# colinvaz/nmf-toolbox

Measured on AMD Instinct MI355X. Metric: NMF multiplicative-update iterations/s, higher is better.
Workload: dtype f32; 1 GPU; nmf.m kl MU, V=16384x65536 K=256 fp32, V column-sharded over 1 GPU(s); m=16384, n=65536, K=256, T=1, divergence=kl

## Files before the change

### nmf_toolbox_amd/build.py

```python
from __future__ import annotations

import os
import subprocess
import sys
from concurrent.futures import ThreadPoolExecutor

HERE = os.path.dirname(os.path.abspath(__file__))
CSRC = os.path.join(HERE, "csrc")
INC = os.path.join(os.path.dirname(HERE), "include")
OUT = os.path.join(HERE, "libnmfx.so")
SOURCES = ["fused_cnmf_a.hip", "fused_cnmf_b.hip", "fused_cnmf_c.hip", "fused_cnmf_e.hip", "fused_cnmf_d.hip", "fused_cnmf_g.hip", "fused_cnmf_f.hip", "gemm_pipe_edge.hip", "gemm_pipe.hip", "gemm.hip", "fused_k224_256.hip", "fused_rag_k224_256.hip", "fused_k128_192.hip", "fused_rag_k128_192.hip", "fused_k32_96.hip", "fused_rag_k32_96.hip", "fused.hip", "aux.hip", "projfunc.hip", "small_mm.hip", "gemm64.hip", "engine.hip", "host_io.hip", "blocking.hip", "sc.hip", "sc64.hip", "multi_sc.hip", "rccl_backend.hip", "cmfwisa.hip", "seminmf.hip"]
ARCH = "gfx950"


def _torch_lib_dir():
    try:
        import importlib.util
        spec = importlib.util.find_spec("torch")
        if spec and spec.origin:
            d = os.path.join(os.path.dirname(spec.origin), "lib")
            if os.path.exists(os.path.join(d, "libamdhip64.so")):
                return d
    except Exception:
        pass
    return None


def _deps(src, incdirs, seen=None):
    import re
    seen = set() if seen is None else seen
    if src in seen or not os.path.exists(src):
        return seen
    seen.add(src)
    with open(src) as f:
        for name in re.findall(r'^\s*#\s*include\s*"([^"]+)"', f.read(), re.M):
            for d in [os.path.dirname(src)] + incdirs:
                cand = os.path.join(d, name)
                if os.path.exists(cand):
                    _deps(cand, incdirs, seen)
                    break
    return seen


def _newer(src_list, target):
    if not os.path.exists(target):
        return True
    t = os.path.getmtime(target)
    return any(os.path.getmtime(s) > t for s in src_list)


VARIANTS = {
    "r5": ["-DNMFX_KL_MODE=0", "-DNMFX_G2_VEC=0", "-DNMFX_G1_ASM=0"],
    "kl1": ["-DNMFX_KL_MODE=1", "-DNMFX_G2_VEC=0", "-DNMFX_G1_ASM=0"],
    "kl2": ["-DNMFX_KL_MODE=2", "-DNMFX_G2_VEC=0", "-DNMFX_G1_ASM=0"],
    "kl2g2": ["-DNMFX_KL_MODE=2", "-DNMFX_G2_VEC=1", "-DNMFX_G1_ASM=0"],
}


def build(force: bool = False, verbose: bool = False, sanitize: bool = False, variant: str = "") -> str:
    srcs = [os.path.join(CSRC, s) for s in SOURCES if os.path.exists(os.path.join(CSRC, s))]
    objdir = os.path.join(CSRC, "_obj_asan" if sanitize else ("_obj_" + variant if variant else "_obj"))
    out = os.path.join(HERE, "libnmfx_asan.so") if sanitize else (os.path.join(HERE, "libnmfx_%s.so" % variant) if variant else OUT)
    vdefs = VARIANTS[variant] if variant else []
    san = ["-fsanitize=address,undefined", "-fno-sanitize=function", "-fno-gpu-sanitize", "-fno-sanitize-recover=undefined", "-Xarch_host", "-g", "-Xarch_host", "-fno-omit-frame-pointer"] if sanitize else []
    os.makedirs(objdir, exist_ok=True)
    hipcc = os.environ.get("HIPCC", "/opt/rocm/bin/hipcc")

    def compile_one(src):
        obj = os.path.join(objdir, os.path.basename(src) + ".o")
        if force or _newer(sorted(_deps(src, [CSRC, INC])) + [os.path.abspath(__file__)], obj):
            cmd = [hipcc, f"--offload-arch={ARCH}", "-O3", "-std=c++17", "-fPIC", "-Wall", "-Werror=uninitialized", "-Wno-pass-failed"] + san + vdefs + [
                   "-I", INC, "-I", CSRC, "-c", src, "-o", obj]
            if os.path.basename(src).startswith("fused_"):
                cmd[3:3] = ["-mllvm", "-pragma-unroll-threshold=1000000"]
            if verbose:
                print(" ".join(cmd), flush=True)
            subprocess.check_call(cmd)
        return obj

    with ThreadPoolExecutor(max_workers=min(len(srcs), 8)) as ex:
        objs = list(ex.map(compile_one, srcs))
    if force or _newer(objs, out):
        tl = _torch_lib_dir()
        libdirs = ([tl] if tl else []) + ["/opt/rocm/lib"]
        if sanitize:
            cmd = ["/opt/rocm/lib/llvm/bin/clang++", "-shared", "-fsanitize=address,undefined", "-fno-sanitize=function", "-o", out] + objs
        else:
            cmd = ["g++", "-shared", "-o", out] + objs
# ... 34 lines not shown
```

### nmf_toolbox_amd/csrc/fused_kernel.h

```cpp
#pragma once
#include "nmfx_internal.h"

namespace nmfx {

typedef float f32x16 __attribute__((ext_vector_type(16)));
typedef float f32x2 __attribute__((ext_vector_type(2)));

typedef int i32x4 __attribute__((ext_vector_type(4)));

constexpr int FT_ROWS = 128;
constexpr int FT_C = 64;

__device__ __forceinline__ f32x2 pk_mul_t(f32x2 a, f32x2 b) { f32x2 d; asm("s_nop 0\n\tv_pk_mul_f32 %0, %1, %2" : "=v"(d) : "v"(a), "v"(b)); return d; }
__device__ __forceinline__ f32x2 pk_fma_t(f32x2 a, f32x2 b, f32x2 c) { f32x2 d; asm("s_nop 0\n\tv_pk_fma_f32 %0, %1, %2, %3" : "=v"(d) : "v"(a), "v"(b), "v"(c)); return d; }
__device__ __forceinline__ f32x2 pk_fnma(f32x2 a, f32x2 b, f32x2 c) { f32x2 d; asm("v_pk_fma_f32 %0, %1, %2, %3 neg_lo:[1,0,0] neg_hi:[1,0,0]" : "=v"(d) : "v"(a), "v"(b), "v"(c)); return d; }
__device__ __forceinline__ f32x2 pk_add(f32x2 a, f32x2 b) { f32x2 d; asm("v_pk_add_f32 %0, %1, %2" : "=v"(d) : "v"(a), "v"(b)); return d; }

__device__ __forceinline__ void mfma_settle_full(f32x16 &t) { asm volatile("s_nop 15\n\ts_nop 3" : "+v"(t)); }
__device__ __forceinline__ constexpr int rowmap(int reg, int h) { return (reg & 3) + 8 * (reg >> 2) + 4 * h; }
__device__ __forceinline__ i32x4 make_srd(const void *base, unsigned bytes) {
    const unsigned long long b = (unsigned long long)base;
    i32x4 s;
    s.x = (int)(unsigned)b;
    s.y = (int)((b >> 32) & 0xffffu);
    s.z = (int)bytes;
    s.w = 0x00020000;
    return s;
}

template <int K, bool D_RC, int FUNC, bool DO_G2, int EPI, bool RAG = false, int TT = 1>
__global__ __launch_bounds__(256, ((K <= 128 && FUNC != 4 && FUNC != 5) ? 2 : 1)) void fused_kernel(const FusedParams p) {
    extern __shared__ __attribute__((aligned(16))) float lds[];
    static_assert(TT == 1 || (D_RC && EPI == 0 && (K / TT) % 32 == 0 && K % TT == 0), "TT > 1: W-step form, K/TT a multiple of 32");
    if (p.run_if && *p.run_if == 0) return;
    constexpr int KH = K / TT;
    constexpr int LDY = KH + 4;
    constexpr int NKB = K / 32;
    constexpr int TROWS = FT_C + TT - 1;
    constexpr int BUF = TROWS * LDY;
    constexpr bool NEED_S = FUNC != 0;
    constexpr bool S_IN = FUNC == 7 || FUNC == 8 || FUNC == 10 || FUNC == 19 || FUNC == 20;
    constexpr int MF = FUNC == 8 ? 3 : ((FUNC == 10 || FUNC == 21) ? 1 : FUNC);
    static_assert(!S_IN || (!DO_G2 && D_RC && TT == 1), "partial-S passes: first product only, W-step form");
    constexpr bool DUAL = FUNC == 4 || FUNC == 5;
    constexpr bool NO_V = FUNC == 12 || FUNC == 14;
    constexpr int NVL = (!D_RC && !RAG) ? 8 : 32;
    constexpr bool SWAP = (!D_RC || EPI == 2) && NMFX_G2_VEC;
    static_assert(EPI != 2 || (D_RC && DO_G2 && FUNC == 0 && TT == 1), "EPI 2: W-step form, no first product");
    constexpr bool STB = FUNC == 15 || FUNC == 16;
    constexpr int EF = (FUNC == 15 || FUNC == 19) ? 11 : ((FUNC == 16 || FUNC == 20) ? 13 : FUNC);
    static_assert(!STB || (DO_G2 && D_RC && EPI == 0 && TT == 1), "functors 15 / 16: W-step form with the second product");
    constexpr bool ST2 = (EF == 11 || EF == 13) && !DO_G2 && D_RC;
    constexpr bool BQ = STB || ST2;
    constexpr bool EARLY = !DO_G2 && NEED_S;
    constexpr bool G1A = NMFX_G1_ASM;
    constexpr bool SADD = S_IN && G1A;
    constexpr bool PK = NMFX_KL_MODE == 2 && (MF == 2 || MF == 3) && !DUAL && EF == FUNC;
    constexpr int NU = (DUAL || EF == 11 || EF == 13) ? 8 : ((MF == 3 && NMFX_KL_MODE == 1) ? 6 : 4);
    static_assert(!DUAL || (K <= 192 && TT == 1), "dual-map kernels: K <= 192 (two accumulator sets + the stationary operand must fit 512 VGPRs: 501 at K = 192, spills at 224)");
    constexpr int NG = K / 8;
    constexpr int ROWS_PER_WAVE = (TROWS + 3) / 4;
    auto kofs = [](int kq) constexpr -> int { return (kq / KH) * LDY + (kq % KH); };
    constexpr int G2_KB = KH / 32, G2_NFULL = KH / 128, G2_WREM = G2_KB % 4;
    auto g2_kloc = [](int lb, int i) constexpr -> int {
        if (!NMFX_G2_VEC) return 32 * lb + i;
        return lb < 4 * G2_NFULL ? 128 * (lb / 4) + 4 * i + (lb % 4) : 128 * G2_NFULL + G2_WREM * i + (lb - 4 * G2_NFULL);
    };

    const int tid = threadIdx.x;
    const int lane = tid & 63;
    const int w = __builtin_amdgcn_readfirstlane(tid >> 6);
    const int l31 = lane & 31, h = lane >> 5;
    const long r_wg0 = (long)blockIdx.x * FT_ROWS;
    const long r0 = r_wg0 + 32 * w;
    const long r = r0 + l31;
    const long cbeg = (long)blockIdx.y * p.c_per_split;
    const long cend = cbeg + p.c_per_split < p.Cn ? cbeg + p.c_per_split : p.Cn;
    const int ntiles = RAG ? (int)((cend - cbeg + FT_C - 1) / FT_C) : (int)((cend - cbeg) / FT_C);
    const bool row_ok = !RAG || r < p.R;

    float xreg[NEED_S ? K / 2 : 1];
    if (NEED_S) {
#pragma unroll
        for (int s = 0; s < K / 2; ++s) {
            const int kq = 8 * (s >> 2) + (s & 3);
            xreg[s] = row_ok ? p.X[r * p.xs_r + (long)(kq % KH + 4 * h) * p.xs_k + (long)(TT - 1 - kq / KH) * p.xs_t] : 0.0f;
        }
    }

    f32x16 acc[DO_G2 ? NKB : 1];
    f32x16 acc2[(DO_G2 && DUAL) ? NKB : 1];
#pragma unroll
    for (int kb = 0; kb < (DO_G2 ? NKB : 1); ++kb)
#pragma unroll
        for (int e = 0; e < 16; ++e) acc[kb][e] = 0.0f;
#pragma unroll
    for (int kb = 0; kb < ((DO_G2 && DUAL) ? NKB : 1); ++kb)
#pragma unroll
        for (int e = 0; e < 16; ++e) acc2[kb][e] = 0.0f;
    const float ab_e1 = p.ab_beta - 1.0f, ab_e2 = p.ab_alpha + p.ab_beta - 1.0f, ab_kappa = (p.ab_alpha + p.ab_beta) == 0.0f ? 0.0f : p.ab_beta / (p.ab_alpha + p.ab_beta);

    const float *const Yz = p.Y + (TT == 1 ? (long)blockIdx.z * p.yz_stride : 0L);
    const int ystride = p.y_stride > 0 ? (int)p.y_stride : K;
    const unsigned lds0 = (unsigned)(uintptr_t)(__attribute__((address_space(3))) float *)lds;
    const unsigned y_voff = (unsigned)lane * 16u;
    auto dma_row = [&](const i32x4 ysrd, int b, int c) {
        const int row = w + 4 * c;
        if (TROWS % 4 != 0 && row >= TROWS) return;
        const unsigned dst = __builtin_amdgcn_readfirstlane(lds0 + (unsigned)((b * BUF + row * LDY) * 4));
        const unsigned soff = __builtin_amdgcn_readfirstlane((unsigned)(row * (TT > 1 ? KH : ystride) * 4));
        unsigned keep;
        if (lane < KH / 4)
            asm volatile("s_mov_b32 %0, m0\n\ts_mov_b32 m0, %3\n\ts_nop 0\n\tbuffer_load_dwordx4 %1, %2, %4 offen lds\n\ts_mov_b32 m0, %0"
                         : "=&s"(keep) : "v"(y_voff), "s"(ysrd), "s"(dst), "s"(soff) : "memory");
    };
    auto tile_rows = [&](int t) -> int {
        if (!RAG) return FT_C;
        const long left = cend - (cbeg + (long)t * FT_C);
        return left >= FT_C ? FT_C : (left > 0 ? (int)left : 0);
    };
    auto y_srd = [&](int t) {
        if (TT > 1) return make_srd(p.Y + (cbeg + (long)t * FT_C - (TT - 1)) * KH, (unsigned)((tile_rows(t) + TT - 1) * KH * 4));
        return make_srd(Yz + (cbeg + (long)t * FT_C) * ystride, (unsigned)(tile_rows(t) > 0 ? ((tile_rows(t) - 1) * ystride + K) * 4 : 0));
    };

    float d[32];
    const unsigned d_voff = D_RC ? (unsigned)((r + 4 * h * p.ldd) * 4) : (unsigned)((p.ldd * (r - r_wg0) + 4 * h) * 4);
    const long wg_rows = RAG ? (p.R - r_wg0 < FT_ROWS ? p.R - r_wg0 : (long)FT_ROWS) : (long)FT_ROWS;
    const __amdgpu_buffer_rsrc_t d_srd_fixed =
        __builtin_amdgcn_make_buffer_rsrc((void *)(p.D + p.ldd * r_wg0), 0, (int)(unsigned)(wg_rows * p.ldd * 4), 0x00020000);
    auto d_srd = [&](int t) {
        if (D_RC) return __builtin_amdgcn_make_buffer_rsrc((void *)(p.D + p.ldd * (cbeg + (long)t * FT_C)), 0, (int)(unsigned)(tile_rows(t) * p.ldd * 4), 0x00020000);
        return d_srd_fixed;
    };
    auto load_d_piece = [&](const __amdgpu_buffer_rsrc_t srd, int t, int i) {
        if (FUNC == 7 || NO_V) return;
        if (D_RC) {
#pragma unroll
            for (int u = 0; u < 2; ++u) {
                const int e = 2 * i + u, jb = e >> 4, reg = e & 15;
                const int soff = (int)(p.ldd * (32 * jb + (reg & 3) + 8 * (reg >> 2)) * 4);
                d[e] = __builtin_bit_cast(float, __builtin_amdgcn_raw_buffer_load_b32(srd, d_voff, soff, 0));
            }
        } else if ((i & 1) == 0) {
            const int f = i >> 1, jb = f >> 2, q = f & 3;
            const int soff = (int)((cbeg + (long)t * FT_C + 32 * jb + 8 * q) * 4);
            if (!RAG) {
                typedef unsigned u32x4 __attribute__((ext_vector_type(4)));
                typedef float f32x4 __attribute__((ext_vector_type(4)));
                const f32x4 q4 = __builtin_bit_cast(f32x4, (u32x4)__builtin_amdgcn_raw_buffer_load_b128(srd, d_voff, soff, 0));
                d[jb * 16 + 4 * q + 0] = q4.x; d[jb * 16 + 4 * q + 1] = q4.y; d[jb * 16 + 4 * q + 2] = q4.z; d[jb * 16 + 4 * q + 3] = q4.w;
                return;
            }
#pragma unroll
            for (int e = 0; e < 4; ++e)
                d[jb * 16 + 4 * q + e] = __builtin_bit_cast(float, __builtin_amdgcn_raw_buffer_load_b32(srd, d_voff, soff + 4 * e, 0));
        }
    };

    float sin_[S_IN ? 32 : 1];
    float sin_n[(S_IN && NMFX_G1_ASM) ? 32 : 1];
    auto s_srd = [&](int t) {
        return __builtin_amdgcn_make_buffer_rsrc((void *)(p.Sin ? p.Sin + p.ldd * (cbeg + (long)t * FT_C) : p.D), 0, p.Sin ? (int)(unsigned)(tile_rows(t) * p.ldd * 4) : 0, 0x00020000);
    };
    auto load_s_piece = [&](const __amdgpu_buffer_rsrc_t srd, int i, bool nxt = false) {
#pragma unroll
        for (int u = 0; u < 2; ++u) {
            const int e = 2 * i + u, jb = e >> 4, reg = e & 15;
            const float sv = __builtin_bit_cast(float, __builtin_amdgcn_raw_buffer_load_b32(srd, d_voff, (int)(p.ldd * (32 * jb + (reg & 3) + 8 * (reg >> 2)) * 4), 0));
            if (S_IN && NMFX_G1_ASM && nxt) sin_n[(S_IN && NMFX_G1_ASM) ? e : 0] = sv;
            else sin_[S_IN ? e : 0] = sv;
        }
    };

    double cost = 0.0;
    if (ntiles > 0) {
        const i32x4 ys = y_srd(0);
#pragma unroll
        for (int c = 0; c < ROWS_PER_WAVE; ++c) dma_row(ys, 0, c);
        const __amdgpu_buffer_rsrc_t ds0 = d_srd(0);
#pragma unroll
        for (int i = 0; i < 16; ++i) load_d_piece(ds0, 0, i);
        if (S_IN) {
            const __amdgpu_buffer_rsrc_t ss0 = s_srd(0);
#pragma unroll
            for (int i = 0; i < 16; ++i) load_s_piece(ss0, i);
        }
    }
    for (int t = 0; t < ntiles; ++t) {
        const int b = t & 1;
        const int tn = t + 1 < ntiles ? t + 1 : t;
        {
            if (EARLY || STB) { if (t == 0) asm volatile("s_waitcnt vmcnt(0)" ::: "memory"); }
            else if (NEED_S && !NO_V) {
                if (NVL == 32) asm volatile("s_waitcnt vmcnt(32)" ::: "memory");
                else asm volatile("s_waitcnt vmcnt(8)" ::: "memory");
            }
            else asm volatile("s_waitcnt vmcnt(0)" ::: "memory");
            __syncthreads();
        }
        const float *Yt = lds + b * BUF;
        const i32x4 ysn = y_srd(tn);
        const __amdgpu_buffer_rsrc_t dsn = d_srd(tn);
        const __amdgpu_buffer_rsrc_t ssn = S_IN ? s_srd(tn) : dsn;
        int dma_c = 0;
        auto dma_some = [&](int upto) {
#pragma unroll
            for (int c = 0; c < ROWS_PER_WAVE; ++c)
                if (c >= dma_c && c < upto) dma_row(ysn, b ^ 1, c);
            dma_c = upto > dma_c ? upto : dma_c;
        };

        f32x16 sacc[2];
        f32x16 sacc2[DUAL ? 2 : 1];
        float bq[BQ ? 2 : 1][BQ ? 16 : 1];
        const __amdgpu_buffer_rsrc_t rs_b = STB ? __builtin_amdgcn_make_buffer_rsrc((void *)(p.Rout + p.ldd * (cbeg + (long)t * FT_C)), 0, (int)(unsigned)(tile_rows(t) * p.ldd * 4), 0x00020000)
                                                : d_srd_fixed;
        float tc = 0.0f;
        float ts = 0.0f;
        f32x2 tc2[2] = {{0.0f, 0.0f}, {0.0f, 0.0f}}, ts2[2] = {{0.0f, 0.0f}, {0.0f, 0.0f}};
        f32x2 es2[2], er2[2], eq2[2];
        const int cvh = RAG ? tile_rows(t) - 4 * h : 0;
        float es[2], er[2], eq[2];
        auto emap_u = [&](int jb, int reg, int u) {
            const int sl = reg & 1;
            if (FUNC == 7) return;
            const float v = NO_V ? 0.0f : d[jb * 16 + reg];
            const bool live = !RAG || (32 * jb + (reg & 3) + 8 * (reg >> 2)) < cvh;
            if (FUNC == 4) {
                if (u == 0) { es[sl] = sacc[jb][reg]; er[sl] = __builtin_amdgcn_rcpf(es[sl]); }
                if (u == 1) eq[sl] = v * er[sl];
                if (u == 2) sacc2[jb][reg] = live ? er[sl] : 0.0f;
                if (u == 3) sacc[jb][reg] = live ? eq[sl] * er[sl] : 0.0f;
                if (u == 4) er[sl] = __builtin_amdgcn_logf(eq[sl]);
                if (u == 5) tc = live ? tc + eq[sl] : tc;
                if (u == 6) tc = live ? fmaf(-0.6931471805599453f, er[sl], tc) : tc;
                if (u == 5 || u == 6) asm volatile("" : "+v"(tc));
            } else if (FUNC == 5) {
                if (u == 0) { es[sl] = sacc[jb][reg]; er[sl] = __builtin_amdgcn_fmed3f(__builtin_amdgcn_logf(es[sl]), -3.0e38f, 3.0e38f); }
                if (u == 1) eq[sl] = ab_e1 * er[sl];
                if (u == 2) eq[sl] = __builtin_amdgcn_exp2f(eq[sl]);
                if (u == 3) er[sl] = __builtin_amdgcn_exp2f(ab_e2 * er[sl]);
                if (u == 4) { eq[sl] = v * eq[sl]; sacc[jb][reg] = live ? eq[sl] : 0.0f; }
                if (u == 5) sacc2[jb][reg] = live ? er[sl] : 0.0f;
                if (u == 6) eq[sl] = fmaf(-ab_kappa, er[sl], eq[sl]);
                if (u == 7) { tc = live ? fmaf(es[sl], eq[sl], tc) : tc; asm volatile("" : "+v"(tc)); }
            } else if (EF == 11) {
                if (u == 0) { es[sl] = sacc[jb][reg]; er[sl] = __builtin_amdgcn_rcpf(es[sl]); }
                if (u == 1) eq[sl] = v * er[sl];
                if (BQ && u == 2) bq[BQ ? jb : 0][BQ ? reg : 0] = er[sl];
                if (u == 3) sacc[jb][reg] = live ? eq[sl] * er[sl] : 0.0f;
                if (u == 4) er[sl] = __builtin_amdgcn_logf(eq[sl]);
                if (u == 5) tc = live ? tc + eq[sl] : tc;
// ... 67 lines not shown
                    sacc[jb][reg + 2 * pr + 1] = lv[2 * pr + 1] ? er2[pr].y : 0.0f;
                }
                if (MF == 3) {
                    eq2[0] = pk_fnma(er2[0], es2[0], es2[0]);
                    eq2[1] = pk_fnma(er2[1], es2[1], es2[1]);
                    er2[0].x = __builtin_amdgcn_logf(er2[0].x); er2[0].y = __builtin_amdgcn_logf(er2[0].y);
                }
            }
            if (b == 2 && MF == 3) {
                er2[1].x = __builtin_amdgcn_logf(er2[1].x); er2[1].y = __builtin_amdgcn_logf(er2[1].y);
#pragma unroll
                for (int pr = 0; pr < 2; ++pr) {
                    const f32x2 t = pk_fma_t(vv[pr], er2[pr], tc2[pr]);
                    const f32x2 u = pk_add(ts2[pr], eq2[pr]);
                    if (RAG) {
                        tc2[pr].x = lv[2 * pr] ? t.x : tc2[pr].x; tc2[pr].y = lv[2 * pr + 1] ? t.y : tc2[pr].y;
                        ts2[pr].x = lv[2 * pr] ? u.x : ts2[pr].x; ts2[pr].y = lv[2 * pr + 1] ? u.y : ts2[pr].y;
                    } else { tc2[pr] = t; ts2[pr] = u; }
                    asm volatile("" : "+v"(tc2[pr]), "+v"(ts2[pr]));
                }
            }
        };
        auto emap_fill = [&](int jb, int i, int M) {
            if (PK) {
#pragma unroll
                for (int q = 0; q < 4 * NBD; ++q)
                    if ((2 * q + 1) * M / (8 * NBD) == i) emap_burst(jb, q / NBD, q % NBD);
                return;
            }
            const int q0 = 16 * NU * i / M, q1 = 16 * NU * (i + 1) / M;
#pragma unroll
            for (int q = q0; q < q1; ++q) emap_u(jb, q / NU, q % NU);
        };
        auto g1_read = [&](int jb, int g) { return *reinterpret_cast<const float4 *>(Yt + (32 * jb + l31) * LDY + kofs(8 * g) + 4 * h); };
        if (NEED_S) {
#pragma unroll
            for (int jb = 0; jb < 2; ++jb)
#pragma unroll
                for (int e = 0; e < 16; ++e) sacc[jb][e] = (S_IN && !SADD) ? sin_[S_IN ? jb * 16 + e : 0] : 0.0f;
            float4 a_cur = g1_read(0, 0);
#pragma unroll
            for (int ph = 0; ph < 2; ++ph) {
#pragma unroll
                for (int g = 0; g < NG; ++g) {
                    float4 a_nxt = a_cur;
                    if (g + 1 < NG) a_nxt = g1_read(ph, g + 1);
                    else if (ph == 0) a_nxt = g1_read(1, 0);
                    auto one = [&](int e, float av) {
#if NMFX_G1_ASM
                      if (G1A) {
                        constexpr bool XA = K / 2 + (DO_G2 ? (DUAL ? 2 : 1) * NKB * 16 : 0) <= 256;
                        const bool first = g == 0 && e == 0 && (!S_IN || SADD);
                        if (ph == 1 && g == 0 && e == 0) {
                            if (XA) {
                                if (first) asm volatile("v_mfma_f32_32x32x2_f32 %0, %2, %3, 0\n\ts_nop 3" : "=&v"(sacc[1]), "+v"(sacc[0]) : "v"(av), "a"(xreg[0]));
                                else asm volatile("v_mfma_f32_32x32x2_f32 %0, %2, %3, %0\n\ts_nop 3" : "+v"(sacc[1]), "+v"(sacc[0]) : "v"(av), "a"(xreg[0]));
                            } else {
                                if (first) asm volatile("v_mfma_f32_32x32x2_f32 %0, %2, %3, 0\n\ts_nop 3" : "=&v"(sacc[1]), "+v"(sacc[0]) : "v"(av), "v"(xreg[0]));
                                else asm volatile("v_mfma_f32_32x32x2_f32 %0, %2, %3, %0\n\ts_nop 3" : "+v"(sacc[1]), "+v"(sacc[0]) : "v"(av), "v"(xreg[0]));
                            }
                            if (SADD) {
#pragma unroll
                                for (int q = 0; q < 16; ++q) sacc[0][q] += sin_[S_IN ? q : 0];
                            }
                        } else if (XA) {
                            if (first) asm volatile("v_mfma_f32_32x32x2_f32 %0, %1, %2, 0" : "=&v"(sacc[ph]) : "v"(av), "a"(xreg[4 * g + e]));
                            else asm volatile("v_mfma_f32_32x32x2_f32 %0, %1, %2, %0" : "+v"(sacc[ph]) : "v"(av), "a"(xreg[4 * g + e]));
                        } else {
                            if (first) asm volatile("v_mfma_f32_32x32x2_f32 %0, %1, %2, 0" : "=&v"(sacc[ph]) : "v"(av), "v"(xreg[4 * g + e]));
                            else asm volatile("v_mfma_f32_32x32x2_f32 %0, %1, %2, %0" : "+v"(sacc[ph]) : "v"(av), "v"(xreg[4 * g + e]));
                        }
                      } else
#endif
                        sacc[ph] = __builtin_amdgcn_mfma_f32_32x32x2f32(av, xreg[4 * g + e], sacc[ph], 0, 0, 0);
                        if (ph == 1) emap_fill(0, 4 * g + e, 4 * NG);
                        if (ph == 0 && e == 0) dma_some(((g + 1) * ROWS_PER_WAVE + NG - 1) / NG);
                        if (S_IN && ph == 1 && 4 * g + e < 16) load_s_piece(ssn, 4 * g + e, true);
                        __builtin_amdgcn_sched_barrier(0);
                    };
                    one(0, a_cur.x); one(1, a_cur.y); one(2, a_cur.z); one(3, a_cur.w);
                    a_cur = a_nxt;
                }
            }
        } else {
#pragma unroll
            for (int reg = 0; reg < 16; ++reg) emap_u(0, reg, 0);
#pragma unroll
            for (int reg = 0; reg < 16; ++reg) emap_u(1, reg, 0);
        }
#if NMFX_G1_ASM
        if (NEED_S && G1A && !DO_G2) {
            mfma_settle_full(sacc[1]);
            if (SADD) {
#pragma unroll
                for (int q = 0; q < 16; ++q) sacc[1][q] += sin_[S_IN ? 16 + q : 0];
            }
        }
#endif
        if (DO_G2) {
            if (STB) asm volatile("s_waitcnt vmcnt(0)" ::: "memory");
            auto g2_read = [&](int jb, int reg, float (&y)[NKB]) {
                if (NMFX_G2_VEC) {
                    const float *yrow = Yt + (32 * jb + rowmap(reg, h)) * LDY;
#pragma unroll
                    for (int pb = 0; pb < TT; ++pb) {
#pragma unroll
                        for (int c = 0; c < G2_NFULL; ++c) {
                            const float4 t4 = *reinterpret_cast<const float4 *>(yrow + pb * LDY + 128 * c + 4 * l31);
                            y[pb * G2_KB + 4 * c + 0] = t4.x; y[pb * G2_KB + 4 * c + 1] = t4.y; y[pb * G2_KB + 4 * c + 2] = t4.z; y[pb * G2_KB + 4 * c + 3] = t4.w;
                        }
                        if (G2_WREM == 2) {
                            const float2 t2 = *reinterpret_cast<const float2 *>(yrow + pb * LDY + 128 * G2_NFULL + 2 * l31);
                            y[pb * G2_KB + 4 * G2_NFULL + 0] = t2.x; y[pb * G2_KB + 4 * G2_NFULL + 1] = t2.y;
                        } else {
#pragma unroll
                            for (int j = 0; j < G2_WREM; ++j) y[pb * G2_KB + 4 * G2_NFULL + j] = yrow[pb * LDY + 128 * G2_NFULL + G2_WREM * l31 + j];
                        }
                    }
                    return;
                }
                const float *yrow = Yt + (32 * jb + rowmap(reg, h)) * LDY + l31;
#pragma unroll
                for (int kb = 0; kb < NKB; ++kb) y[kb] = yrow[kofs(32 * kb)];
            };
            float y_cur[NKB], y_nxt[NKB];
            g2_read(0, 0, y_cur);
#pragma unroll
            for (int st = 0; st < 32; ++st) {
                const int jb = st >> 4, reg = st & 15;
                if (st + 1 < 32) g2_read((st + 1) >> 4, (st + 1) & 15, y_nxt);
                const float rr = sacc[jb][reg];
                const float rr2 = DUAL ? sacc2[jb][reg] : 0.0f;
#pragma unroll
                for (int kb = 0; kb < NKB; ++kb) {
#if NMFX_G1_ASM
                    if (NEED_S && G1A && st == 0 && kb == 0) {
                        if (SWAP) asm volatile("v_mfma_f32_32x32x2_f32 %0, %2, %3, %0\n\ts_nop 3" : "+a"(acc[0]), "+v"(sacc[1]) : "v"(rr), "v"(y_cur[0]));
                        else asm volatile("v_mfma_f32_32x32x2_f32 %0, %2, %3, %0\n\ts_nop 3" : "+a"(acc[0]), "+v"(sacc[1]) : "v"(y_cur[0]), "v"(rr));
                    } else
#endif
                    acc[kb] = SWAP ? __builtin_amdgcn_mfma_f32_32x32x2f32(rr, y_cur[kb], acc[kb], 0, 0, 0) : __builtin_amdgcn_mfma_f32_32x32x2f32(y_cur[kb], rr, acc[kb], 0, 0, 0);
                    if (jb == 0 && NEED_S) emap_fill(1, (reg * NKB + kb) * (DUAL ? 2 : 1), 16 * NKB * (DUAL ? 2 : 1));
                    if (kb == 0 && !NEED_S) dma_some((st + 1) * ROWS_PER_WAVE / 24 < ROWS_PER_WAVE ? (st + 1) * ROWS_PER_WAVE / 24 : ROWS_PER_WAVE);
                    if (kb == NKB / 2 && jb == (NEED_S ? 1 : 0)) load_d_piece(dsn, tn, reg);
                    if (STB && kb == 1 && (jb == 1 || reg >= 8)) {
                        auto put = [&](int j2, int r2) {
                            const float bv = bq[STB ? j2 : 0][STB ? r2 : 0];
                            if (row_ok) __builtin_amdgcn_raw_buffer_store_b32(__builtin_bit_cast(unsigned, bv), rs_b, d_voff, (int)(p.ldd * (32 * j2 + (r2 & 3) + 8 * (r2 >> 2)) * 4), 0);
                        };
                        if (jb == 0) { put(0, 2 * (reg - 8)); put(0, 2 * (reg - 8) + 1); }
                        else put(1, reg);
                    }
                    __builtin_amdgcn_sched_barrier(0);
                    if (DUAL) {
                        acc2[kb] = SWAP ? __builtin_amdgcn_mfma_f32_32x32x2f32(rr2, y_cur[kb], acc2[kb], 0, 0, 0) : __builtin_amdgcn_mfma_f32_32x32x2f32(y_cur[kb], rr2, acc2[kb], 0, 0, 0);
                        if (jb == 0) emap_fill(1, (reg * NKB + kb) * 2 + 1, 32 * NKB);
                        __builtin_amdgcn_sched_barrier(0);
                    }
                }
#pragma unroll
                for (int kb = 0; kb < NKB; ++kb) y_cur[kb] = y_nxt[kb];
            }
        } else {
            if (S_IN) asm volatile("s_waitcnt vmcnt(32)" ::: "memory");
            else if (EARLY) asm volatile("s_waitcnt vmcnt(0)" ::: "memory");
            if (PK) {
#pragma unroll
                for (int q = 0; q < 4 * NBD; ++q) emap_burst(1, q / NBD, q % NBD);
            } else {
#pragma unroll
                for (int reg = 0; reg < 16; ++reg)
#pragma unroll
                    for (int u = 0; u < NU; ++u) emap_u(1, reg, u);
            }
            if (D_RC && ((MF >= 2 && MF <= 3) || FUNC == 7 || FUNC == 1 || FUNC == 21 || ST2) && p.Rout) {
                const __amdgpu_buffer_rsrc_t rs = __builtin_amdgcn_make_buffer_rsrc((void *)(p.Rout + p.ldd * (cbeg + (long)t * FT_C)), 0, (int)(unsigned)(tile_rows(t) * p.ldd * 4), 0x00020000);
                if (row_ok) {
#pragma unroll
                    for (int e = 0; e < 32; ++e) {
                        const int jb = e >> 4, reg = e & 15;
                        const float rv = sacc[jb][reg];
                        __builtin_amdgcn_raw_buffer_store_b32(__builtin_bit_cast(unsigned, rv), rs, d_voff, (int)(p.ldd * (32 * jb + (reg & 3) + 8 * (reg >> 2)) * 4), 0);
                    }
                }
            }
            if (ST2 && p.Rout2) {
                const __amdgpu_buffer_rsrc_t rs2 = __builtin_amdgcn_make_buffer_rsrc((void *)(p.Rout2 + p.ldd * (cbeg + (long)t * FT_C)), 0, (int)(unsigned)(tile_rows(t) * p.ldd * 4), 0x00020000);
                if (row_ok) {
#pragma unroll
                    for (int e = 0; e < 32; ++e) {
                        const int jb = e >> 4, reg = e & 15;
                        const float bv = bq[BQ ? jb : 0][BQ ? reg : 0];
                        __builtin_amdgcn_raw_buffer_store_b32(__builtin_bit_cast(unsigned, bv), rs2, d_voff, (int)(p.ldd * (32 * jb + (reg & 3) + 8 * (reg >> 2)) * 4), 0);
                    }
                }
            }
#pragma unroll
            for (int i = 0; i < 16; ++i) load_d_piece(dsn, tn, i);
        }
        dma_some(ROWS_PER_WAVE);
        if (SADD) {
#pragma unroll
            for (int e = 0; e < 32; ++e) sin_[S_IN ? e : 0] = sin_n[(S_IN && NMFX_G1_ASM) ? e : 0];
        }
        if (MF == 3 && NMFX_KL_MODE == 2) cost += row_ok ? ((double)tc2[0].x + (double)tc2[0].y + (double)tc2[1].x + (double)tc2[1].y) * 0.6931471805599453 + ((double)ts2[0].x + (double)ts2[0].y + (double)ts2[1].x + (double)ts2[1].y) : 0.0;
        else if (MF == 3 && NMFX_KL_MODE == 1) cost += row_ok ? (double)tc * 0.6931471805599453 + (double)ts : 0.0;
        else cost += row_ok ? (double)tc : 0.0;
    }

    auto e_kloc = [&](int kb, int reg) -> int { return g2_kloc(kb % G2_KB, SWAP ? l31 : rowmap(reg, h)); };
    auto e_row = [&](int reg) -> long { return SWAP ? r0 + rowmap(reg, h) : r; };
    auto e_ok = [&](int reg) -> bool { return !RAG || e_row(reg) < p.R; };
    if (DO_G2) {
        if (EPI == 0 || EPI == 2) {
            float *out = p.out + (long)blockIdx.y * p.slab_stride + (TT == 1 ? (long)blockIdx.z * p.oz_stride : 0L);
#pragma unroll
            for (int q = 0; q < 16 * NKB; ++q) {
                const int kb = SWAP ? q % NKB : q / 16, reg = SWAP ? q / NKB : q % 16;
                if (e_ok(reg)) {
                    const long oi = e_row(reg) * p.os_r + (long)e_kloc(kb, reg) * p.os_k + (long)(TT - 1 - kb / G2_KB) * p.os_t;
                    out[oi] = acc[kb][reg];
                    if (DUAL) p.out2[(long)blockIdx.y * p.slab_stride + oi] = acc2[kb][reg];
                }
            }
        } else {
            bool lines_done = false;
            if (SWAP && !DUAL && G2_NFULL > 0 && p.H64 && !p.fix && !p.sqrt_rule) {
                lines_done = true;
#pragma unroll
                for (int reg = 0; reg < 16; ++reg) {
                    if (!e_ok(reg)) continue;
#pragma unroll
                    for (int c = 0; c < G2_NFULL; ++c) {
                        const int k0 = 128 * c + 4 * l31;
                        const long idx0 = (long)k0 + (long)K * e_row(reg);
                        double hv[4], dn[4];
#pragma unroll
                        for (int o = 0; o < 4; ++o) hv[o] = p.H64[idx0 + o];
#pragma unroll
                        for (int o = 0; o < 4; ++o) dn[o] = (p.den ? (double)p.den[idx0 + o] : p.denvec[k0 + o]) + (p.lam ? (double)p.lam[k0 + o] : 0.0);
#pragma unroll
                        for (int o = 0; o < 4; ++o) hv[o] = hv[o] * ((double)acc[4 * c + o][reg] / fmax(dn[o], 2.220446049250313e-16));
#pragma unroll
                        for (int o = 0; o < 4; ++o) p.H64[idx0 + o] = hv[o];
#pragma unroll
                        for (int o = 0; o < 4; ++o) p.Hio[idx0 + o] = (float)hv[o];
                    }
                }
            }
#pragma unroll
            for (int q = 0; q < 16 * NKB; ++q) {
                    const int kb = SWAP ? q % NKB : q / 16, reg = SWAP ? q / NKB : q % 16;
                    if (lines_done && kb < 4 * G2_NFULL) continue;
                    const int k = e_kloc(kb, reg);
                    if (!e_ok(reg) || (p.fix && p.fix[k])) continue;
                    const long idx = (long)k + (long)K * e_row(reg);
                    const float lam = p.lam ? p.lam[k] : 0.0f;
                    if (p.H64) {
                        const double hv = p.H64[idx];
                        double hn;
                        if (p.sqrt_rule) hn = sqrt(hv * (double)acc[kb][reg]);
                        else if (DUAL) {
                            double gn = (double)acc[kb][reg], gp = (double)acc2[kb][reg];
                            if (p.inv_exp != 1.0f) { gn = pow(gn, (double)p.inv_exp); gp = pow(gp, (double)p.inv_exp); }
                            hn = hv * (gn / fmax(gp + (double)lam, 2.220446049250313e-16));
                        } else hn = hv * ((double)acc[kb][reg] / fmax((p.den ? (double)p.den[idx] : p.denvec[k]) + (double)lam, 2.220446049250313e-16));
                        p.H64[idx] = hn;
                        p.Hio[idx] = (float)hn;
                        continue;
                    }
                    if (p.sqrt_rule) { p.Hio[idx] = sqrtf(p.Hio[idx] * acc[kb][reg]); continue; }
                    if (DUAL) {
                        float gn = acc[kb][reg], gp = acc2[kb][reg];
                        if (p.inv_exp != 1.0f) { gn = powf(gn, p.inv_exp); gp = powf(gp, p.inv_exp); }
                        p.Hio[idx] = p.Hio[idx] * (gn / fmaxf(gp + lam, NMFX_EPS_F));
                        continue;
                    }
                    const float den = p.den ? p.den[idx] : (float)p.denvec[k];
                    p.Hio[idx] = p.Hio[idx] * (acc[kb][reg] / fmaxf(den + lam, NMFX_EPS_F));
                }
        }
// ... 14 lines not shown
```

### nmf_toolbox_amd/csrc/nmfx_internal.h

```cpp
#pragma once
#include <hip/hip_runtime.h>
#include <stddef.h>
#include <stdint.h>

#include "nmfx.h"

#define NMFX_EPS_F 2.220446049250313e-16f

namespace nmfx {

void set_error(const char *fmt, ...);
#define NMFX_HIP(call)                                                                    \
    do {                                                                                  \
        hipError_t e_ = (call);                                                           \
        if (e_ != hipSuccess) {                                                           \
            nmfx::set_error("%s failed: %s (%s:%d)", #call, hipGetErrorString(e_), __FILE__, __LINE__); \
            return NMFX_ERR_HIP;                                                          \
        }                                                                                 \
    } while (0)

#define TRY(x) do { nmfx_status s_ = (x); if (s_ != NMFX_OK) return s_; } while (0)

struct LdsAttrOnce {
    int set_bytes[64] = {};
// ... 62 lines not shown
    int accumulate;
    int clamp0;
    int store_c;
    int epi;
    int cost_div;
    float cost_alpha, cost_beta;
    const float *Vref;
    long ldv;
    double *cost_partials;
    long cost_ncols;
    int splitk;
    long slab_stride;
    long kc_per_split;
    int zbatch;
    long zA_off, zB_off;
    int zB_lim, zB_tstride;
};
bool gemm_pipe_eligible(const GemmParams &p);

nmfx_status launch_gemm(hipStream_t st, const GemmParams &p, long *blocks_out = nullptr);
nmfx_status gemm_auto(hipStream_t st, GemmParams p, void *scratch, size_t scratch_bytes);
int gemm_pick_split(long M, long N, long Kc);
long gemm_grid_blocks(long M, long N);
size_t gemm_scratch_bytes(long M, long N, long Kc);

#ifndef NMFX_KL_MODE
#define NMFX_KL_MODE 2
#endif
#ifndef NMFX_G2_VEC
#define NMFX_G2_VEC 1
#endif
#ifndef NMFX_G1_ASM
#define NMFX_G1_ASM 1
#endif
constexpr bool KL_CONSISTENT_COST = NMFX_KL_MODE != 0;
struct FusedParams {
    const float *X;
    long xs_r, xs_k;
    int T;
    long xs_t, os_t;
    const float *Y;
    long y_stride;
    int nz;
    long yz_stride, oz_stride;
    const float *D;
    long ldd;
    long R, Cn;
    long c_per_split;
    int K;
    float *out;
    float *Rout2;
    float *Rout;
    const float *Sin;
    float *out2;
    float ab_alpha, ab_beta;
    float inv_exp;
    long slab_stride, os_r, os_k;
    double *cost_partials;
    float *Hio;
    const float *den;
    const double *denvec;
    const float *lam;
    const uint8_t *fix;
    int sqrt_rule;
    double *H64;
    const int *run_if;
// ... 127 lines not shown
```

Before: 65.83 iterations/s.

## Overlap tile-seam work in fused KL kernel and pipeline H epilogue loads

```diff
diff --git a/nmf_toolbox_amd/build.py b/nmf_toolbox_amd/build.py
--- a/nmf_toolbox_amd/build.py
+++ b/nmf_toolbox_amd/build.py
@@ -54,6 +54,10 @@
     "kl1": ["-DNMFX_KL_MODE=1", "-DNMFX_G2_VEC=0", "-DNMFX_G1_ASM=0"],
     "kl2": ["-DNMFX_KL_MODE=2", "-DNMFX_G2_VEC=0", "-DNMFX_G1_ASM=0"],
     "kl2g2": ["-DNMFX_KL_MODE=2", "-DNMFX_G2_VEC=1", "-DNMFX_G1_ASM=0"],
+    "cost_off": ["-DNMFX_SEAM_COST=0"],
+    "addr_off": ["-DNMFX_SEAM_ADDR=0"],
+    "sync_off": ["-DNMFX_SEAM_SYNC=0"],
+    "epi_off": ["-DNMFX_EPI_PIPE=0"],
 }
 
 
diff --git a/nmf_toolbox_amd/csrc/fused_kernel.h b/nmf_toolbox_amd/csrc/fused_kernel.h
--- a/nmf_toolbox_amd/csrc/fused_kernel.h
+++ b/nmf_toolbox_amd/csrc/fused_kernel.h
@@ -1,5 +1,6 @@
 #pragma once
 #include "nmfx_internal.h"
+#include <type_traits>
 
 namespace nmfx {
 
@@ -58,6 +59,10 @@
     constexpr bool PK = NMFX_KL_MODE == 2 && (MF == 2 || MF == 3) && !DUAL && EF == FUNC;
     constexpr int NU = (DUAL || EF == 11 || EF == 13) ? 8 : ((MF == 3 && NMFX_KL_MODE == 1) ? 6 : 4);
     static_assert(!DUAL || (K <= 192 && TT == 1), "dual-map kernels: K <= 192 (two accumulator sets + the stationary operand must fit 512 VGPRs: 501 at K = 192, spills at 224)");
+    constexpr bool TWO = DO_G2 && NEED_S && !STB;
+    constexpr bool DEFC = NMFX_SEAM_COST && TWO && PK && MF == 3;
+    constexpr bool ADDR = NMFX_SEAM_ADDR && TWO && !RAG;
+    constexpr bool ESYNC = NMFX_SEAM_SYNC && TWO;
     constexpr int NG = K / 8;
     constexpr int ROWS_PER_WAVE = (TROWS + 3) / 4;
     auto kofs = [](int kq) constexpr -> int { return (kq / KH) * LDY + (kq % KH); };
@@ -104,10 +109,11 @@
     const int ystride = p.y_stride > 0 ? (int)p.y_stride : K;
     const unsigned lds0 = (unsigned)(uintptr_t)(__attribute__((address_space(3))) float *)lds;
     const unsigned y_voff = (unsigned)lane * 16u;
-    auto dma_row = [&](const i32x4 ysrd, int b, int c) {
+    const unsigned ldsw0 = __builtin_amdgcn_readfirstlane(lds0 + (unsigned)(w * LDY * 4));
+    auto dma_row = [&](const i32x4 ysrd, unsigned ldsb, int c, int cd, bool own) {
         const int row = w + 4 * c;
         if (TROWS % 4 != 0 && row >= TROWS) return;
-        const unsigned dst = __builtin_amdgcn_readfirstlane(lds0 + (unsigned)((b * BUF + row * LDY) * 4));
+        const unsigned dst = __builtin_amdgcn_readfirstlane(own ? ldsb + (unsigned)(4 * cd * LDY * 4) : lds0 + (unsigned)(((int)ldsb * BUF + row * LDY) * 4));
         const unsigned soff = __builtin_amdgcn_readfirstlane((unsigned)(row * (TT > 1 ? KH : ystride) * 4));
         unsigned keep;
         if (lane < KH / 4)
@@ -119,18 +125,25 @@
         const long left = cend - (cbeg + (long)t * FT_C);
         return left >= FT_C ? FT_C : (left > 0 ? (int)left : 0);
     };
+    auto y_rec = [&](int t) -> unsigned {
+        if (TT > 1) return (unsigned)((tile_rows(t) + TT - 1) * KH * 4);
+        return (unsigned)(tile_rows(t) > 0 ? ((tile_rows(t) - 1) * ystride + K) * 4 : 0);
+    };
     auto y_srd = [&](int t) {
-        if (TT > 1) return make_srd(p.Y + (cbeg + (long)t * FT_C - (TT - 1)) * KH, (unsigned)((tile_rows(t) + TT - 1) * KH * 4));
-        return make_srd(Yz + (cbeg + (long)t * FT_C) * ystride, (unsigned)(tile_rows(t) > 0 ? ((tile_rows(t) - 1) * ystride + K) * 4 : 0));
-    };
+        if (TT > 1) return make_srd(p.Y + (cbeg + (long)t * FT_C - (TT - 1)) * KH, y_rec(t));
+        return make_srd(Yz + (cbeg + (long)t * FT_C) * ystride, y_rec(t));
+    };
+    const long y_step = (long)FT_C * (TT > 1 ? KH : ystride) * 4;
 
     float d[32];
     const unsigned d_voff = D_RC ? (unsigned)((r + 4 * h * p.ldd) * 4) : (unsigned)((p.ldd * (r - r_wg0) + 4 * h) * 4);
     const long wg_rows = RAG ? (p.R - r_wg0 < FT_ROWS ? p.R - r_wg0 : (long)FT_ROWS) : (long)FT_ROWS;
     const __amdgpu_buffer_rsrc_t d_srd_fixed =
         __builtin_amdgcn_make_buffer_rsrc((void *)(p.D + p.ldd * r_wg0), 0, (int)(unsigned)(wg_rows * p.ldd * 4), 0x00020000);
+    auto d_ptr = [&](int t) -> const float * { return p.D + p.ldd * (cbeg + (long)t * FT_C); };
+    auto d_rec = [&](int t) -> int { return (int)(unsigned)(tile_rows(t) * p.ldd * 4); };
     auto d_srd = [&](int t) {
-        if (D_RC) return __builtin_amdgcn_make_buffer_rsrc((void *)(p.D + p.ldd * (cbeg + (long)t * FT_C)), 0, (int)(unsigned)(tile_rows(t) * p.ldd * 4), 0x00020000);
+        if (D_RC) return __builtin_amdgcn_make_buffer_rsrc((void *)d_ptr(t), 0, d_rec(t), 0x00020000);
         return d_srd_fixed;
     };
     auto load_d_piece = [&](const __amdgpu_buffer_rsrc_t srd, int t, int i) {
@@ -173,11 +186,30 @@
         }
     };
 
+    auto rows_wait = [&]() {
+        if (NEED_S && !NO_V) {
+            static_assert(NVL == 32 || NVL == 8, "rows_wait: one s_waitcnt per value of NVL");
+            if (NVL == 32) asm volatile("s_waitcnt vmcnt(32)" ::: "memory");
+            else asm volatile("s_waitcnt vmcnt(8)" ::: "memory");
+        } else asm volatile("s_waitcnt vmcnt(0)" ::: "memory");
+    };
+    auto g1_read_at = [&](const float *Yb, int jb, int g) { return *reinterpret_cast<const float4 *>(Yb + (32 * jb + l31) * LDY + kofs(8 * g) + 4 * h); };
+    const int t1 = ntiles > 1 ? 1 : 0;
+    i32x4 ys_c = y_srd(t1);
+    const float *dp_c = d_ptr(t1);
+    int dr_c = d_rec(t1);
+    unsigned ldsn_c = ldsw0 + (unsigned)(BUF * 4);
+    int yoff_c = 0;
+    float4 a_first = {0.0f, 0.0f, 0.0f, 0.0f};
+    f32x2 tc2[2] = {{0.0f, 0.0f}, {0.0f, 0.0f}}, ts2[2] = {{0.0f, 0.0f}, {0.0f, 0.0f}};
+    f32x2 ptc2[2] = {{0.0f, 0.0f}, {0.0f, 0.0f}}, pts2[2] = {{0.0f, 0.0f}, {0.0f, 0.0f}};
+    double dca = 0.0, dcb = 0.0;
+    constexpr double LN2 = 0.6931471805599453;
     double cost = 0.0;
     if (ntiles > 0) {
         const i32x4 ys = y_srd(0);
 #pragma unroll
-        for (int c = 0; c < ROWS_PER_WAVE; ++c) dma_row(ys, 0, c);
+        for (int c = 0; c < ROWS_PER_WAVE; ++c) dma_row(ys, 0u, c, c, false);
         const __amdgpu_buffer_rsrc_t ds0 = d_srd(0);
 #pragma unroll
         for (int i = 0; i < 16; ++i) load_d_piece(ds0, 0, i);
@@ -185,6 +217,11 @@
             const __amdgpu_buffer_rsrc_t ss0 = s_srd(0);
 #pragma unroll
             for (int i = 0; i < 16; ++i) load_s_piece(ss0, i);
+        }
+        if (ESYNC) {
+            rows_wait();
+            __syncthreads();
+            a_first = g1_read_at(lds, 0, 0);
         }
     }
     for (int t = 0; t < ntiles; ++t) {
@@ -192,22 +229,26 @@
         const int tn = t + 1 < ntiles ? t + 1 : t;
         {
             if (EARLY || STB) { if (t == 0) asm volatile("s_waitcnt vmcnt(0)" ::: "memory"); }
-            else if (NEED_S && !NO_V) {
-                if (NVL == 32) asm volatile("s_waitcnt vmcnt(32)" ::: "memory");
-                else asm volatile("s_waitcnt vmcnt(8)" ::: "memory");
-            }
-            else asm volatile("s_waitcnt vmcnt(0)" ::: "memory");
-            __syncthreads();
-        }
-        const float *Yt = lds + b * BUF;
-        const i32x4 ysn = y_srd(tn);
-        const __amdgpu_buffer_rsrc_t dsn = d_srd(tn);
+            else if (!ESYNC) rows_wait();
+            if (!ESYNC) __syncthreads();
+        }
+        const float *Yt = lds + (ADDR ? yoff_c : b * BUF);
+        const i32x4 ysn = ADDR ? ys_c : y_srd(tn);
+        const __amdgpu_buffer_rsrc_t dsn = ADDR ? (D_RC ? __builtin_amdgcn_make_buffer_rsrc((void *)dp_c, 0, dr_c, 0x00020000) : d_srd_fixed) : d_srd(tn);
+        const unsigned ldsn = ldsn_c;
         const __amdgpu_buffer_rsrc_t ssn = S_IN ? s_srd(tn) : dsn;
+        unsigned dma_dst = ldsn;
         int dma_c = 0;
         auto dma_some = [&](int upto) {
 #pragma unroll
             for (int c = 0; c < ROWS_PER_WAVE; ++c)
-                if (c >= dma_c && c < upto) dma_row(ysn, b ^ 1, c);
+                if (c >= dma_c && c < upto) {
+                    if (ADDR) {
+                        dma_row(ysn, dma_dst, c, 0, true);
+                        dma_dst += (unsigned)(4 * LDY * 4);
+                        asm volatile("" : "+s"(dma_dst));
+                    } else dma_row(ysn, (unsigned)(b ^ 1), c, c, false);
+                }
             dma_c = upto > dma_c ? upto : dma_c;
         };
 
@@ -218,7 +259,7 @@
                                                 : d_srd_fixed;
         float tc = 0.0f;
         float ts = 0.0f;
-        f32x2 tc2[2] = {{0.0f, 0.0f}, {0.0f, 0.0f}}, ts2[2] = {{0.0f, 0.0f}, {0.0f, 0.0f}};
+        if (!DEFC) { tc2[0] = tc2[1] = ts2[0] = ts2[1] = f32x2{0.0f, 0.0f}; }
         f32x2 es2[2], er2[2], eq2[2];
         const int cvh = RAG ? tile_rows(t) - 4 * h : 0;
         float es[2], er[2], eq[2];
@@ -352,13 +393,38 @@
 #pragma unroll
             for (int q = q0; q < q1; ++q) emap_u(jb, q / NU, q % NU);
         };
-        auto g1_read = [&](int jb, int g) { return *reinterpret_cast<const float4 *>(Yt + (32 * jb + l31) * LDY + kofs(8 * g) + 4 * h); };
+        auto g1_read = [&](int jb, int g) { return g1_read_at(Yt, jb, g); };
+        auto g2_read = [&](int jb, int reg, float (&y)[NKB]) {
+            if (NMFX_G2_VEC) {
+                const float *yrow = Yt + (32 * jb + rowmap(reg, h)) * LDY;
+#pragma unroll
+                for (int pb = 0; pb < TT; ++pb) {
+#pragma unroll
+                    for (int c = 0; c < G2_NFULL; ++c) {
+                        const float4 t4 = *reinterpret_cast<const float4 *>(yrow + pb * LDY + 128 * c + 4 * l31);
+                        y[pb * G2_KB + 4 * c + 0] = t4.x; y[pb * G2_KB + 4 * c + 1] = t4.y; y[pb * G2_KB + 4 * c + 2] = t4.z; y[pb * G2_KB + 4 * c + 3] = t4.w;
+                    }
+                    if (G2_WREM == 2) {
+                        const float2 t2 = *reinterpret_cast<const float2 *>(yrow + pb * LDY + 128 * G2_NFULL + 2 * l31);
+                        y[pb * G2_KB + 4 * G2_NFULL + 0] = t2.x; y[pb * G2_KB + 4 * G2_NFULL + 1] = t2.y;
+                    } else {
+#pragma unroll
+                        for (int j = 0; j < G2_WREM; ++j) y[pb * G2_KB + 4 * G2_NFULL + j] = yrow[pb * LDY + 128 * G2_NFULL + G2_WREM * l31 + j];
+                    }
+                }
+                return;
+            }
+            const float *yrow = Yt + (32 * jb + rowmap(reg, h)) * LDY + l31;
+#pragma unroll
+            for (int kb = 0; kb < NKB; ++kb) y[kb] = yrow[kofs(32 * kb)];
+        };
+        float y_cur[NKB], y_nxt[NKB];
         if (NEED_S) {
 #pragma unroll
             for (int jb = 0; jb < 2; ++jb)
 #pragma unroll
                 for (int e = 0; e < 16; ++e) sacc[jb][e] = (S_IN && !SADD) ? sin_[S_IN ? jb * 16 + e : 0] : 0.0f;
-            float4 a_cur = g1_read(0, 0);
+            float4 a_cur = ESYNC ? a_first : g1_read(0, 0);
 #pragma unroll
             for (int ph = 0; ph < 2; ++ph) {
 #pragma unroll
@@ -395,6 +461,14 @@
                         sacc[ph] = __builtin_amdgcn_mfma_f32_32x32x2f32(av, xreg[4 * g + e], sacc[ph], 0, 0, 0);
                         if (ph == 1) emap_fill(0, 4 * g + e, 4 * NG);
                         if (ph == 0 && e == 0) dma_some(((g + 1) * ROWS_PER_WAVE + NG - 1) / NG);
+                        if (DEFC && ph == 0 && e == 2 && g < 3) {
+                            if (g == 0) asm volatile("" : "+v"(ptc2[0]), "+v"(ptc2[1]));
+                            if (g == 1) asm volatile("" : "+v"(pts2[0]), "+v"(pts2[1]));
+                            if (g == 0) { dca = (double)ptc2[0].x + (double)ptc2[0].y + (double)ptc2[1].x + (double)ptc2[1].y; asm volatile("" : "+v"(dca)); }
+                            if (g == 1) { dcb = (double)pts2[0].x + (double)pts2[0].y + (double)pts2[1].x + (double)pts2[1].y; asm volatile("" : "+v"(dcb)); }
+                            if (g == 2) { cost += row_ok ? dca * LN2 + dcb : 0.0; asm volatile("" : "+v"(cost)); }
+                        }
+                        if (ESYNC && ph == 1 && g == NG - 1 && e == 1) g2_read(0, 0, y_cur);
                         if (S_IN && ph == 1 && 4 * g + e < 16) load_s_piece(ssn, 4 * g + e, true);
                         __builtin_amdgcn_sched_barrier(0);
                     };
@@ -419,32 +493,8 @@
 #endif
         if (DO_G2) {
             if (STB) asm volatile("s_waitcnt vmcnt(0)" ::: "memory");
-            auto g2_read = [&](int jb, int reg, float (&y)[NKB]) {
-                if (NMFX_G2_VEC) {
-                    const float *yrow = Yt + (32 * jb + rowmap(reg, h)) * LDY;
-#pragma unroll
-                    for (int pb = 0; pb < TT; ++pb) {
-#pragma unroll
-                        for (int c = 0; c < G2_NFULL; ++c) {
-                            const float4 t4 = *reinterpret_cast<const float4 *>(yrow + pb * LDY + 128 * c + 4 * l31);
-                            y[pb * G2_KB + 4 * c + 0] = t4.x; y[pb * G2_KB + 4 * c + 1] = t4.y; y[pb * G2_KB + 4 * c + 2] = t4.z; y[pb * G2_KB + 4 * c + 3] = t4.w;
-                        }
-                        if (G2_WREM == 2) {
-                            const float2 t2 = *reinterpret_cast<const float2 *>(yrow + pb * LDY + 128 * G2_NFULL + 2 * l31);
-                            y[pb * G2_KB + 4 * G2_NFULL + 0] = t2.x; y[pb * G2_KB + 4 * G2_NFULL + 1] = t2.y;
-                        } else {
-#pragma unroll
-                            for (int j = 0; j < G2_WREM; ++j) y[pb * G2_KB + 4 * G2_NFULL + j] = yrow[pb * LDY + 128 * G2_NFULL + G2_WREM * l31 + j];
-                        }
-                    }
-                    return;
-                }
-                const float *yrow = Yt + (32 * jb + rowmap(reg, h)) * LDY + l31;
-#pragma unroll
-                for (int kb = 0; kb < NKB; ++kb) y[kb] = yrow[kofs(32 * kb)];
-            };
-            float y_cur[NKB], y_nxt[NKB];
-            g2_read(0, 0, y_cur);
+            if (!(ESYNC && NEED_S)) g2_read(0, 0, y_cur);
+            constexpr int VKB = ESYNC ? (NKB > 1 ? 1 : 0) : NKB / 2;
 #pragma unroll
             for (int st = 0; st < 32; ++st) {
                 const int jb = st >> 4, reg = st & 15;
@@ -462,7 +512,31 @@
                     acc[kb] = SWAP ? __builtin_amdgcn_mfma_f32_32x32x2f32(rr, y_cur[kb], acc[kb], 0, 0, 0) : __builtin_amdgcn_mfma_f32_32x32x2f32(y_cur[kb], rr, acc[kb], 0, 0, 0);
                     if (jb == 0 && NEED_S) emap_fill(1, (reg * NKB + kb) * (DUAL ? 2 : 1), 16 * NKB * (DUAL ? 2 : 1));
                     if (kb == 0 && !NEED_S) dma_some((st + 1) * ROWS_PER_WAVE / 24 < ROWS_PER_WAVE ? (st + 1) * ROWS_PER_WAVE / 24 : ROWS_PER_WAVE);
-                    if (kb == NKB / 2 && jb == (NEED_S ? 1 : 0)) load_d_piece(dsn, tn, reg);
+                    if (kb == VKB && jb == (NEED_S ? 1 : 0)) load_d_piece(dsn, tn, reg);
+                    if (DEFC && st == 18 && kb == NKB - 1) {
+                        ptc2[0] = tc2[0]; ptc2[1] = tc2[1]; pts2[0] = ts2[0]; pts2[1] = ts2[1];
+                        tc2[0] = tc2[1] = ts2[0] = ts2[1] = f32x2{0.0f, 0.0f};
+                        asm volatile("" : "+v"(ptc2[0]), "+v"(ptc2[1]), "+v"(pts2[0]), "+v"(pts2[1]));
+                        asm volatile("" : "+v"(tc2[0]), "+v"(tc2[1]), "+v"(ts2[0]), "+v"(ts2[1]));
+                    }
+                    if (ADDR && st == 20 && kb == NKB - 1) {
+                        int tq = t;
+                        asm volatile("" : "+s"(tq));
+                        const bool adv = tq + 2 < ntiles;
+                        unsigned long long yb = ((unsigned long long)(unsigned)ys_c.y << 32) | (unsigned)ys_c.x;
+                        yb += adv ? (unsigned long long)y_step : 0ull;
+                        ys_c.x = (int)(unsigned)yb; ys_c.y = (int)(unsigned)(yb >> 32);
+                        dp_c += adv ? p.ldd * FT_C : 0L;
+                        const int bq_ = tq & 1;
+                        ldsn_c = ldsw0 + (unsigned)(bq_ * BUF * 4); yoff_c = (bq_ ^ 1) * BUF;
+                        asm volatile("" : "+s"(ys_c), "+s"(dp_c), "+s"(dr_c), "+s"(ldsn_c), "+s"(yoff_c));
+                    }
+                    if (ESYNC && st == 31 && kb == VKB) {
+                        asm volatile("s_waitcnt lgkmcnt(0)" ::: "memory");
+                        rows_wait();
+                        __syncthreads();
+                        a_first = g1_read_at(lds + (b ^ 1) * BUF, 0, 0);
+                    }
                     if (STB && kb == 1 && (jb == 1 || reg >= 8)) {
                         auto put = [&](int j2, int r2) {
                             const float bv = bq[STB ? j2 : 0][STB ? r2 : 0];
@@ -523,10 +597,13 @@
 #pragma unroll
             for (int e = 0; e < 32; ++e) sin_[S_IN ? e : 0] = sin_n[(S_IN && NMFX_G1_ASM) ? e : 0];
         }
-        if (MF == 3 && NMFX_KL_MODE == 2) cost += row_ok ? ((double)tc2[0].x + (double)tc2[0].y + (double)tc2[1].x + (double)tc2[1].y) * 0.6931471805599453 + ((double)ts2[0].x + (double)ts2[0].y + (double)ts2[1].x + (double)ts2[1].y) : 0.0;
+        if (DEFC) {}
+        else if (MF == 3 && NMFX_KL_MODE == 2) cost += row_ok ? ((double)tc2[0].x + (double)tc2[0].y + (double)tc2[1].x + (double)tc2[1].y) * 0.6931471805599453 + ((double)ts2[0].x + (double)ts2[0].y + (double)ts2[1].x + (double)ts2[1].y) : 0.0;
         else if (MF == 3 && NMFX_KL_MODE == 1) cost += row_ok ? (double)tc * 0.6931471805599453 + (double)ts : 0.0;
         else cost += row_ok ? (double)tc : 0.0;
     }
+
+    if (DEFC) cost += row_ok ? ((double)ptc2[0].x + (double)ptc2[0].y + (double)ptc2[1].x + (double)ptc2[1].y) * LN2 + ((double)pts2[0].x + (double)pts2[0].y + (double)pts2[1].x + (double)pts2[1].y) : 0.0;
 
     auto e_kloc = [&](int kb, int reg) -> int { return g2_kloc(kb % G2_KB, SWAP ? l31 : rowmap(reg, h)); };
     auto e_row = [&](int reg) -> long { return SWAP ? r0 + rowmap(reg, h) : r; };
@@ -547,6 +624,75 @@
             bool lines_done = false;
             if (SWAP && !DUAL && G2_NFULL > 0 && p.H64 && !p.fix && !p.sqrt_rule) {
                 lines_done = true;
+#if NMFX_EPI_PIPE
+              if (!RAG) {
+                constexpr int NCH = G2_NFULL > 0 ? G2_NFULL : 1, NIT = 16 * NCH, DEPTH = K <= 128 ? 2 : 6;
+                float lmf[NCH][4];
+                double dvec[NCH][4];
+#pragma unroll
+                for (int c = 0; c < NCH; ++c)
+#pragma unroll
+                    for (int o = 0; o < 4; ++o) { lmf[c][o] = 0.0f; dvec[c][o] = 0.0; }
+                if (p.lam) {
+#pragma unroll
+                    for (int c = 0; c < NCH; ++c)
+#pragma unroll
+                        for (int o = 0; o < 4; ++o) lmf[c][o] = p.lam[128 * c + 4 * l31 + o];
+                }
+                if (!p.den) {
+#pragma unroll
+                    for (int c = 0; c < NCH; ++c)
+#pragma unroll
+                        for (int o = 0; o < 4; ++o) dvec[c][o] = p.denvec[128 * c + 4 * l31 + o];
+                }
+                double lamv[NCH][4];
+#pragma unroll
+                for (int c = 0; c < NCH; ++c)
+#pragma unroll
+                    for (int o = 0; o < 4; ++o) lamv[c][o] = p.den ? (double)lmf[c][o] : fmax(dvec[c][o] + (double)lmf[c][o], 2.220446049250313e-16);
+                auto run = [&](auto matrix_den) {
+                    constexpr bool MD = decltype(matrix_den)::value;
+                    double hq[DEPTH][4];
+                    float dq[MD ? DEPTH : 1][4];
+                    auto idx_of = [&](int i) -> long { return (long)(128 * (i % NCH) + 4 * l31) + (long)K * e_row(i / NCH); };
+                    auto request = [&](int i) {
+                        if (!e_ok(i / NCH)) return;
+                        const long idx0 = idx_of(i);
+#pragma unroll
+                        for (int o = 0; o < 4; ++o) hq[i % DEPTH][o] = p.H64[idx0 + o];
+                        if (MD) {
+#pragma unroll
+                            for (int o = 0; o < 4; ++o) dq[MD ? i % DEPTH : 0][o] = p.den[idx0 + o];
+                        }
+                    };
+#pragma unroll
+                    for (int i = 0; i < (DEPTH < NIT ? DEPTH : NIT); ++i) request(i);
+#pragma unroll
+                    for (int i = 0; i < NIT; ++i) {
+                        const int reg = i / NCH, c = i % NCH;
+                        double hv[4];
+                        if (e_ok(reg)) {
+                            const long idx0 = idx_of(i);
+#pragma unroll
+                            for (int o = 0; o < 4; ++o) asm volatile("" : "+a"(acc[4 * c + o]));
+#pragma unroll
+                            for (int o = 0; o < 4; ++o) {
+                                const double dn = MD ? fmax((double)dq[MD ? i % DEPTH : 0][o] + lamv[c][o], 2.220446049250313e-16) : lamv[c][o];
+                                hv[o] = hq[i % DEPTH][o] * ((double)acc[4 * c + o][reg] / dn);
+                            }
+#pragma unroll
+                            for (int o = 0; o < 4; ++o) p.H64[idx0 + o] = hv[o];
+#pragma unroll
+                            for (int o = 0; o < 4; ++o) p.Hio[idx0 + o] = (float)hv[o];
+                        }
+                        if (i + DEPTH < NIT) request(i + DEPTH);
+                    }
+                };
+                if (p.den) run(std::true_type{});
+                else run(std::false_type{});
+              } else
+#endif
+              {
 #pragma unroll
                 for (int reg = 0; reg < 16; ++reg) {
                     if (!e_ok(reg)) continue;
@@ -567,6 +713,7 @@
                         for (int o = 0; o < 4; ++o) p.Hio[idx0 + o] = (float)hv[o];
                     }
                 }
+              }
             }
 #pragma unroll
             for (int q = 0; q < 16 * NKB; ++q) {
diff --git a/nmf_toolbox_amd/csrc/nmfx_internal.h b/nmf_toolbox_amd/csrc/nmfx_internal.h
--- a/nmf_toolbox_amd/csrc/nmfx_internal.h
+++ b/nmf_toolbox_amd/csrc/nmfx_internal.h
@@ -118,6 +118,18 @@
 #endif
 #ifndef NMFX_G1_ASM
 #define NMFX_G1_ASM 1
+#endif
+#ifndef NMFX_SEAM_COST
+#define NMFX_SEAM_COST 1
+#endif
+#ifndef NMFX_SEAM_ADDR
+#define NMFX_SEAM_ADDR 1
+#endif
+#ifndef NMFX_SEAM_SYNC
+#define NMFX_SEAM_SYNC 1
+#endif
+#ifndef NMFX_EPI_PIPE
+#define NMFX_EPI_PIPE 1
 #endif
 constexpr bool KL_CONSISTENT_COST = NMFX_KL_MODE != 0;
 struct FusedParams {
```

After: 66.26 iterations/s (median of 6 runs). Within noise of the previous version (+0.6%).
